# inferflow/inferflow

Measured on AMD Instinct MI355X. Metric: decode tokens/sec, Llama-2-7B Q4 batch=1 greedy (whole job), higher is better.
Workload: dtype i8 (Q8 activations x Q4_B32T1A weights, i32 dot, f32 scale, f16 I/O); 1 GPU; llama2_7b decode, Q4_B32T1A weights + F16 lm_head, F16 KV cache, batch 1 greedy, 16-token prompt, context 21..1851; parallelism=single, weights_bytes=4309647360

## Files before the change

inferflow_amd/csrc/ifa_decode_attn.h:

```cpp
#pragma once
#include "ifa_decode_kernels.h"

namespace ifa {

struct DecAttnParams {
    const half_t *q;
    const half_t *k_new;
    const half_t *v_new;
    uint8_t *kcache, *vcache;
    const int *state;
    const float *rope_tab;
    int heads, kv_heads, kv_q8;
    float kq_scale;
    int rope_order, rope_cols;
    int alibi, alibi_base, alibi_total;
    half_t *out;
    int max_ctx;
    int8_t *xq;
    long long *trace;
    const void *batch_rows;
    int q_stride;
};
struct DecAttnBatchRow { const uint8_t *kc, *vc; int n_ctx, pad; };

// ... 34 lines not shown
    float c[IFA_ATTN_NACC];
    __device__ __forceinline__ ScoreAcc() {
#pragma unroll
        for (int i = 0; i < IFA_ATTN_NACC; i++) c[i] = 0.0f;
    }
    __device__ __forceinline__ void add2(int p, half2_t q, half2_t k) {
        if constexpr (IFA_ATTN_NACC == 1) {
            c[0] = __builtin_fmaf((float)q[0], (float)k[0], c[0]);
            c[0] = __builtin_fmaf((float)q[1], (float)k[1], c[0]);
        } else {
            c[p % IFA_ATTN_NACC] = __builtin_amdgcn_fdot2(q, k, c[p % IFA_ATTN_NACC], false);
        }
    }
    __device__ __forceinline__ void add(int d, float q, float k) { c[d % IFA_ATTN_NACC] = __builtin_fmaf(q, k, c[d % IFA_ATTN_NACC]); }
    __device__ __forceinline__ float total() const {
        if constexpr (IFA_ATTN_NACC == 1) return c[0];
        else if constexpr (IFA_ATTN_NACC == 2) return c[0] + c[1];
        else if constexpr (IFA_ATTN_NACC == 4) return (c[0] + c[1]) + (c[2] + c[3]);
        else { float t = c[0]; for (int i = 1; i < IFA_ATTN_NACC; i++) t = t + c[i]; return t; }
    }
};

struct DecAttnFusedIn {
    const unsigned long long *gran;
    unsigned epoch;
    int pos;
    unsigned *err;
    long long timeout_ticks;
    unsigned long long *att_gran;
};

__host__ __device__ inline int att_gran_count(int heads, int hd) { return heads * hd / 4 + 2 * (heads * hd / 32) + heads; }

template <int HD, bool Q8, int PB, bool KT>
struct DecAttnRegs {
    static constexpr int DG = HD / 8, NSPLIT = 256 / DG, VPRE = PB / NSPLIT;
    static constexpr int KBYTES = (HD / 32) * 34;
    static constexpr int KALIGN = HD == 128 ? 8 : (HD == 64 ? 4 : 2);
    uint32_t kreg[Q8 ? 1 : HD / 2];
    uint32_t kq32[(Q8 && KALIGN >= 4) ? KBYTES / 4 : 1];
    uint16_t kq16[(Q8 && KALIGN < 4) ? KBYTES / 2 : 1];
    u32x4 kt[KT ? PB / NSPLIT : 1];
    u32x4 vreg[Q8 ? 1 : VPRE];
    uint32_t vqs[Q8 ? VPRE : 1], vqc[Q8 ? VPRE : 1][2];
    float rope_cs, rope_sn;
    half_t q_in, k_in, v_in;
};

template <int HD, bool Q8, bool BATCH, int PB, bool KT, bool FUSED, int PHASE = 0>
__device__ __forceinline__ void dec_attn_body(char *smem, const half_t *pq, const uint8_t *pkc, const uint8_t *pvc, int pheads, int pkvh,
                                              const DecAttnParams &P, const int h_in, const DecAttnFusedIn &F, DecAttnRegs<HD, Q8, PB, KT> &R)
{
    int pos_b = 0;
    if constexpr (FUSED) pos_b = F.pos;
    if constexpr (BATCH) {
        const DecAttnBatchRow br = reinterpret_cast<const DecAttnBatchRow *>(P.batch_rows)[blockIdx.y];
        pkc = br.kc; pvc = br.vc; pos_b = br.n_ctx - 1;
        pq += (size_t)blockIdx.y * P.q_stride;
    }
#define IFA_GP(T, p) ((const __attribute__((address_space(1))) T *)(p))
    uint8_t *const kcw = BATCH ? const_cast<uint8_t *>(pkc) : P.kcache;
    uint8_t *const vcw = BATCH ? const_cast<uint8_t *>(pvc) : P.vcache;
    const float *const rope_tab = BATCH ? P.rope_tab + (size_t)blockIdx.y * HD : P.rope_tab;
    half_t *const outp = BATCH ? P.out + (size_t)blockIdx.y * pheads * HD : P.out;
    static_assert(HD % 8 == 0 && HD <= 128 && (!Q8 || HD % 32 == 0), "head size: multiples of 8 up to 128 (Q8 rows: whole 32-blocks)");
    constexpr int DG = HD / 8;
    constexpr int NSPLIT = 256 / DG;
    half_t *qs = reinterpret_cast<half_t *>(smem);
    half_t *kn = qs + HD;
    half_t *vn = kn + HD;
    float *red = reinterpret_cast<float *>(vn + HD);
    float *opart = red + 16;
    static_assert(!KT || (!Q8 && !BATCH && (DG & (DG - 1)) == 0 && PB % NSPLIT == 0), "K tile through LDS: F16 rows, one query, power-of-two pieces per row");
    static_assert(!(FUSED && BATCH), "the fused tail is a single-query kernel");
    static_assert(PB >= NSPLIT && PB <= DEC_ATTN_MIN_ROWS, "prefetch bucket");
    uint8_t *ktile = reinterpret_cast<uint8_t *>(opart + NSPLIT * HD);
    half_t *S = reinterpret_cast<half_t *>(ktile + (KT ? (size_t)PB * HD * 2 : 0));
    const int h = h_in, tid = threadIdx.x, lane = tid & 63, wave = tid >> 6;
    const int group = pheads / pkvh;
    const int kvh = h / group;
    const bool writer = (h % group) == 0;
    const int kv_dim = pkvh * HD;
    const size_t row_bytes = Q8 ? (size_t)(kv_dim / 32) * 34 : (size_t)kv_dim * 2;
    const size_t head_off = Q8 ? (size_t)((kvh * HD) / 32) * 34 : (size_t)kvh * HD * 2;

    constexpr int KBYTES = (HD / 32) * 34;
    constexpr int KALIGN = HD == 128 ? 8 : (HD == 64 ? 4 : 2);
    auto &kreg = R.kreg; auto &kq32 = R.kq32; auto &kq16 = R.kq16; auto &kt = R.kt; auto &vreg = R.vreg; auto &vqs = R.vqs; auto &vqc = R.vqc;
    float &rope_cs = R.rope_cs, &rope_sn = R.rope_sn;
    half_t &q_in = R.q_in, &k_in = R.k_in, &v_in = R.v_in;
    auto load_k = [&](int j) {
        const uint8_t *rowp = pkc + (size_t)j * row_bytes + head_off;
        if constexpr (Q8) {
// ... 237 lines not shown
    if (n_ctx <= 64) {
        if (wave == 0) {
            if (tr) P.trace[h * 8 + 4] = wall_clock64();
            float e = 0.0f;
            if (tid < n_ctx) e = expf(P.kq_scale * h2f(S[tid]) - lmax);
            const float lsum0 = wave_sum(e);
            const float inv0 = 1.0f / (((lsum0 + 0.0f) + 0.0f) + 0.0f);
            if (tid < n_ctx) S[tid] = f2h(h2f(f2h(e)) * inv0);
        }
        __syncthreads();
    } else {
    if (lane == 0) red[wave] = lmax;
    __syncthreads();
    if (tr) P.trace[h * 8 + 4] = wall_clock64();
    const float mx = fmaxf(fmaxf(red[0], red[1]), fmaxf(red[2], red[3]));
    float lsum = 0.0f;
    for (int j = tid; j < n_ctx; j += 256) {
        const float e = expf(P.kq_scale * h2f(S[j]) - mx);
        lsum += e;
        S[j] = f2h(e);
    }
    lsum = wave_sum(lsum);
    if (lane == 0) red[4 + wave] = lsum;
    __syncthreads();
    const float inv = 1.0f / (((red[4] + red[5]) + red[6]) + red[7]);
    for (int j = tid; j < n_ctx; j += 256) S[j] = f2h(h2f(S[j]) * inv);
    __syncthreads();
    }
    if (tr) P.trace[h * 8 + 5] = wall_clock64();

    float o[8];
#pragma unroll
    for (int i = 0; i < 8; i++) o[i] = 0.0f;
    auto acc_v = [&](float pj, const u32x4 vv) {
        const half8_t v8 = __builtin_bit_cast(half8_t, vv);
#pragma unroll
        for (int e = 0; e < 8; e++) o[e] = __builtin_fmaf(pj, (float)v8[e], o[e]);
    };
    auto acc_new = [&](float pj) {
#pragma unroll
        for (int e = 0; e < 8; e++) o[e] = __builtin_fmaf(pj, h2f(vn[dg * 8 + e]), o[e]);
    };
    auto acc_q8w = [&](float pj, uint16_t scb, uint16_t c0, uint16_t c1, uint16_t c2, uint16_t c3) {
        const half_t sch = __builtin_bit_cast(half_t, scb);
        const half2_t sc2 = {sch, sch};
        half2_t v01, v23, v45, v67;
        q8x4_dequant_h((uint32_t)c0 | ((uint32_t)c1 << 16), sc2, v01, v23);
        q8x4_dequant_h((uint32_t)c2 | ((uint32_t)c3 << 16), sc2, v45, v67);
        o[0] = __builtin_fmaf(pj, (float)v01[0], o[0]); o[1] = __builtin_fmaf(pj, (float)v01[1], o[1]);
        o[2] = __builtin_fmaf(pj, (float)v23[0], o[2]); o[3] = __builtin_fmaf(pj, (float)v23[1], o[3]);
        o[4] = __builtin_fmaf(pj, (float)v45[0], o[4]); o[5] = __builtin_fmaf(pj, (float)v45[1], o[5]);
        o[6] = __builtin_fmaf(pj, (float)v67[0], o[6]); o[7] = __builtin_fmaf(pj, (float)v67[1], o[7]);
    };
    auto acc_q8 = [&](float pj, int j) {
        const auto *blk = IFA_GP(uint16_t, pvc + (size_t)j * row_bytes + head_off + (size_t)(dg / 4) * 34);
        typedef uint32_t u32x2_a2 __attribute__((ext_vector_type(2), aligned(2)));
        const u32x2_a2 cw = *IFA_GP(u32x2_a2, blk + 1 + (dg % 4) * 4);
        acc_q8w(pj, blk[0], (uint16_t)(cw[0] & 0xFFFFu), (uint16_t)(cw[0] >> 16), (uint16_t)(cw[1] & 0xFFFFu), (uint16_t)(cw[1] >> 16));
    };
#pragma unroll
    for (int i = 0; i < VPRE; i++) {
        const int j = sp + NSPLIT * i;
        if (j < n_ctx && vact) {
            const float pj = h2f(S[j]);
            if (j == pos) acc_new(pj);
            else if constexpr (Q8) acc_q8w(pj, (uint16_t)vqs[i], (uint16_t)(vqc[i][0] & 0xFFFFu), (uint16_t)(vqc[i][0] >> 16), (uint16_t)(vqc[i][1] & 0xFFFFu), (uint16_t)(vqc[i][1] >> 16));
            else acc_v(pj, vreg[i]);
        }
    }
    {
        constexpr int TB = 8;
        u32x4 tcur[Q8 ? 1 : TB], tnxt[Q8 ? 1 : TB];
        uint32_t ts_c[Q8 ? TB : 1], tc_c[Q8 ? TB : 1][2], ts_n[Q8 ? TB : 1], tc_n[Q8 ? TB : 1][2];
        const size_t tq_off = head_off + (size_t)(dg / 4) * 34;
        auto tload = [&](u32x4 (&dst)[Q8 ? 1 : TB], uint32_t (&ds)[Q8 ? TB : 1], uint32_t (&dc)[Q8 ? TB : 1][2], int j) {
#pragma unroll
            for (int u = 0; u < TB; u++) {
                const int jr = min(j + u * NSPLIT, n_ctx - 1);
                if constexpr (!Q8) dst[u] = IFA_GP(u32x4, pvc + (size_t)jr * row_bytes + head_off)[dg];
                else {
                    const auto *blk = IFA_GP(uint16_t, pvc + (size_t)jr * row_bytes + tq_off);
                    typedef uint32_t u32x2_a2 __attribute__((ext_vector_type(2), aligned(2)));
                    ds[u] = blk[0];
                    const u32x2_a2 cw = *IFA_GP(u32x2_a2, blk + 1 + (dg % 4) * 4);
                    dc[u][0] = cw[0]; dc[u][1] = cw[1];
                }
            }
        };
        int j = vact ? sp + NSPLIT * VPRE : n_ctx;
        if (j < n_ctx) tload(tcur, ts_c, tc_c, j);
        for (; j < n_ctx; j += TB * NSPLIT) {
            tload(tnxt, ts_n, tc_n, j + TB * NSPLIT);
#pragma unroll
            for (int u = 0; u < TB; u++) {
                const int jj = j + u * NSPLIT;
                if (jj >= n_ctx) break;
                const float pj = h2f(S[jj]);
                if (jj == pos) acc_new(pj);
                else if constexpr (Q8) acc_q8w(pj, (uint16_t)ts_c[u], (uint16_t)(tc_c[u][0] & 0xFFFFu), (uint16_t)(tc_c[u][0] >> 16), (uint16_t)(tc_c[u][1] & 0xFFFFu), (uint16_t)(tc_c[u][1] >> 16));
                else acc_v(pj, tcur[u]);
            }
#pragma unroll
            for (int u = 0; u < TB; u++) {
                if constexpr (Q8) { ts_c[u] = ts_n[u]; tc_c[u][0] = tc_n[u][0]; tc_c[u][1] = tc_n[u][1]; }
                else tcur[u] = tnxt[u];
            }
        }
    }
    if (vact) {
#pragma unroll
        for (int e = 0; e < 8; e++) opart[sp * HD + dg * 8 + e] = o[e];
    }
    if (tr) P.trace[h * 8 + 6] = wall_clock64();
    __syncthreads();
    if (tid < HD) {
        float acc = opart[tid];
        for (int s2 = 1; s2 < NSPLIT; s2++) acc = acc + opart[s2 * HD + tid];
        const half_t yh = f2h(acc);
        outp[(size_t)h * HD + tid] = yh;
        if constexpr (HD % 32 == 0 && !BATCH) { if (P.xq) dec_attn_emit_q8<HD>(P.xq, P.heads * HD, h, tid, yh); }
        if constexpr (FUSED && HD % 32 == 0) {
            if (F.att_gran) {
                const float val = h2f(yh);
                const float mxv = half_wave_max(fabsf(val));
                const float qsc = mxv / 127;
                const int qv = q8_round_div1(val, qsc);
                const int sum = half_wave_sum_i32(qv);
                const int q1 = dpp_xor1(qv), q2 = dpp_xor2(qv), q3 = dpp_xor1(q2);
                const unsigned long long tagw = (unsigned long long)F.epoch << 32;
                const int cols = pheads * HD, nc = cols / 4, nbk = cols / 32;
                if ((tid & 3) == 0) {
                    const uint32_t w4 = (uint32_t)(qv & 0xFF) | ((uint32_t)(q1 & 0xFF) << 8) | ((uint32_t)(q2 & 0xFF) << 16) | ((uint32_t)(q3 & 0xFF) << 24);
                    __hip_atomic_store(F.att_gran + (h * HD + tid) / 4, tagw | w4, __ATOMIC_RELAXED, __HIP_MEMORY_SCOPE_AGENT);
                }
                if ((tid & 31) == 0) {
                    const int blk = (h * HD + tid) >> 5;
                    __hip_atomic_store(F.att_gran + nc + blk, tagw | __builtin_bit_cast(uint32_t, h2f(f2h(qsc))), __ATOMIC_RELAXED, __HIP_MEMORY_SCOPE_AGENT);
                    __hip_atomic_store(F.att_gran + nc + nbk + blk, tagw | __builtin_bit_cast(uint32_t, (float)sum), __ATOMIC_RELAXED, __HIP_MEMORY_SCOPE_AGENT);
                }
                if (tid == 0) __hip_atomic_store(F.att_gran + nc + 2 * nbk + h, tagw | 1u, __ATOMIC_RELAXED, __HIP_MEMORY_SCOPE_AGENT);
            }
        }
    }
    if (tr) P.trace[h * 8 + 7] = wall_clock64();
}

template <int HD, bool Q8, bool BATCH = false, int PB = DEC_ATTN_MIN_ROWS, bool KT = false>
__global__ void __launch_bounds__(256) k_dec_attn(const half_t *pq, const uint8_t *pkc, const uint8_t *pvc, int pheads, int pkvh,
                                                  const DecAttnParams P)
{
    extern __shared__ __attribute__((aligned(16))) char smem[];
    DecAttnRegs<HD, Q8, PB, KT> R;
    dec_attn_body<HD, Q8, BATCH, PB, KT, false>(smem, pq, pkc, pvc, pheads, pkvh, P, (int)blockIdx.x, DecAttnFusedIn{}, R);
}

constexpr int DEC_ATTN_MAX_SPLITS = 32;

struct DecAttnSplitWs {
    half_t *S;
    float *lmax;
    float *opart;
    int nsplits;
};

__device__ __forceinline__ void dec_split_range(int n_ctx, int nsplits, int s, int &j0, int &j1)
{
    const int chunk = ((n_ctx + nsplits - 1) / nsplits + 63) / 64 * 64;
    j0 = min(s * chunk, n_ctx); j1 = min(j0 + chunk, n_ctx);
}

template <int HD, bool Q8>
__global__ void __launch_bounds__(256) k_dec_attn_scores(const DecAttnParams P, const DecAttnSplitWs ws)
{
    __shared__ __attribute__((aligned(16))) half_t qs[HD];
    __shared__ __attribute__((aligned(16))) half_t kn[HD];
// ... 316 lines not shown
```

inferflow_amd/csrc/ifa_decode_qkv_attn.h:

```cpp
#pragma once
#include "ifa_decode_kernels.h"
#include "ifa_decode_attn.h"

namespace ifa {

struct DecQkvAttnExtra {
    unsigned long long *gran;
    const unsigned *epoch;
    unsigned epoch_add;
    unsigned *err;
    int timeout_us;
    int gk;
    int unload;
};

#ifndef IFA_QA_EARLY_KV
#define IFA_QA_EARLY_KV 0
#endif
#ifndef IFA_QA_WARM_ROWS
#define IFA_QA_WARM_ROWS 1
#endif
constexpr int QA_THREADS = 512;

template <int DT, int NJ, int RW, int NORM, int HD, bool Q8, int PB, bool KT, int NP, bool UL = false>
// ... 109 lines not shown
    typename Fmt::X X;
    X.load(L.codes, L.scale, L.xsum, lane, g_nblk);
    {
        float a[RW];
#pragma unroll
        for (int i = 0; i < RW; i++) a[i] = w[i].dot(X);
#pragma unroll
        for (int i = 0; i < RW; i++) a[i] = wave_sum(a[i]);
        float a0 = 0.0f;
#pragma unroll
        for (int i = 0; i < RW; i++) { if (lane == i) a0 = a[i]; }
        const int lr = lane * WGV + lw;
        if (lane < RW && lr < RG) {
            const Row r = locate(lr);
            half_t y = dec_bias(a0, r.b, r.row);
            if (P.pre_scale != 0.0f) y = f2h(h2f(y) * P.pre_scale);
            r.y[r.row] = y;
            __hip_atomic_store(E.gran + r.vrow, ((unsigned long long)epoch << 32) | (unsigned long long)__builtin_bit_cast(uint16_t, y),
                               __ATOMIC_RELAXED, __HIP_MEMORY_SCOPE_AGENT);
        }
    }
    if (A.trace && threadIdx.x == 0) {
        A.trace[(size_t)(A.heads + (int)blockIdx.x) * 8 + 0] = t_kernel;
        A.trace[(size_t)(A.heads + (int)blockIdx.x) * 8 + 1] = wall_clock64();
    }
    if (attn_wg) {
        __syncthreads();
        if (wave >= 4) return;
        dec_attn_body<HD, Q8, false, PB, KT, true, IFA_QA_EARLY_KV ? 2 : 0>(smem, nullptr, A.kcache, A.vcache, A.heads, A.kv_heads, A, head, F, R);
        return;
    }
}

bool dec_qkv_attn_supported(int w_dtype, int cols, int heads, int kv_heads, int head_dim, int num_cus, int *gk_out, int *rw_out);
int dec_qkv_attn_launch(int w_dtype, int norm, bool kv_q8, int pb, bool kt, const DecGemvParams &P, const DecAttnParams &A, const DecQkvAttnExtra &E,
                        int max_ctx, hipStream_t s);
template <int DT>
int dec_qkv_attn_launch_dt(int norm, bool kv_q8, int pb, bool kt, int rw, const DecGemvParams &P, const DecAttnParams &A, const DecQkvAttnExtra &E,
                           int max_ctx, hipStream_t s);

}
```

inferflow_amd/csrc/ifa_dqkvattn_impl.h:

```cpp
#pragma once
#include "ifa_host.h"
#include "ifa_decode_qkv_attn.h"

namespace ifa {

template <int DT, int NJ, int RW, int NORM, bool Q8, int PB, bool KT, bool UL = false>
static int qa_go(const DecGemvParams &P, const DecAttnParams &A, const DecQkvAttnExtra &E, int max_ctx, hipStream_t s)
{
    constexpr int HD = 128;
    auto kern = k_dec_qkv_attn<DT, NJ, RW, NORM, HD, Q8, PB, KT, QA_THREADS / 128, UL>;
    const size_t smem = std::max(xlds_bytes(P.cols), dec_attn_smem(HD, max_ctx, KT ? PB : 0));
    if (smem > (size_t)160 * 1024) return ifa_fail(IFA_ERR_ARG, "fused QKV + attention: %zu bytes of LDS", smem);
    if (smem > 48 * 1024) IFA_HIP_CHECK(hipFuncSetAttribute((const void *)kern, hipFuncAttributeMaxDynamicSharedMemorySize, (int)smem));
    if (A.heads > 255 || A.kv_heads > 255 || E.gk > 0xFFFF) return ifa_fail(IFA_ERR_ARG, "fused QKV + attention: geometry exceeds the packed launch scalar");
    const int pgeo = A.heads | (A.kv_heads << 8) | (E.gk << 16);
    kern<<<dim3((unsigned)(A.kv_heads * E.gk)), dim3(QA_THREADS), smem, s>>>(P.x, P.norm_w, P.norm_b, P.cols, pgeo, P.W0[0], P.W0[1], P.W0[2], P, A, E);
    IFA_LAUNCH_CHECK();
    return IFA_OK;
}

template <int DT, int NJ, int RW, int NORM>
static int qa_pick(bool kv_q8, int pb, bool kt, const DecGemvParams &P, const DecAttnParams &A, const DecQkvAttnExtra &E, int max_ctx, hipStream_t s)
{
    if (kv_q8) {
        if (pb == 64) return qa_go<DT, NJ, RW, NORM, true, 64, false>(P, A, E, max_ctx, s);
        if (pb == 128) return qa_go<DT, NJ, RW, NORM, true, 128, false>(P, A, E, max_ctx, s);
        return qa_go<DT, NJ, RW, NORM, true, 256, false>(P, A, E, max_ctx, s);
    }
    if (kt) {
        if (pb == 64) return qa_go<DT, NJ, RW, NORM, false, 64, true>(P, A, E, max_ctx, s);
        if (pb == 128) return qa_go<DT, NJ, RW, NORM, false, 128, true>(P, A, E, max_ctx, s);
        return qa_go<DT, NJ, RW, NORM, false, 256, true>(P, A, E, max_ctx, s);
    }
    return qa_go<DT, NJ, RW, NORM, false, 256, false>(P, A, E, max_ctx, s);
}

template <int DT, int NJ, int RW, int NORM>
static int qa_pick_ul(bool kv_q8, int pb, bool kt, const DecGemvParams &P, const DecAttnParams &A, const DecQkvAttnExtra &E, int max_ctx, hipStream_t s)
{
    if (pb == 128) {
        if (kv_q8) return qa_go<DT, NJ, RW, NORM, true, 128, false, true>(P, A, E, max_ctx, s);
        if (kt) return qa_go<DT, NJ, RW, NORM, false, 128, true, true>(P, A, E, max_ctx, s);
    }
    if (kv_q8) return qa_go<DT, NJ, RW, NORM, true, 256, false, true>(P, A, E, max_ctx, s);
    if (kt) return qa_go<DT, NJ, RW, NORM, false, 256, true, true>(P, A, E, max_ctx, s);
    return qa_go<DT, NJ, RW, NORM, false, 256, false, true>(P, A, E, max_ctx, s);
}

template <int DT> constexpr int qa_nj(int cols) { return (cols / block_capacity(DT) + 63) / 64; }

template <int DT>
int dec_qkv_attn_launch_dt(int norm, bool kv_q8, int pb, bool kt, int rw, const DecGemvParams &P, const DecAttnParams &A, const DecQkvAttnExtra &E,
                           int max_ctx, hipStream_t s)
{
    constexpr int NJ4K = qa_nj<DT>(4096);
    const int nj = (P.nblk + 63) / 64;
    if (norm != 1) return ifa_fail(IFA_ERR_ARG, "fused QKV + attention: RMS-norm prologue only");
    if (E.unload && nj == NJ4K && rw == 6 && E.gk == 8) return qa_pick_ul<DT, NJ4K, 7, 1>(kv_q8, pb, kt, P, A, E, max_ctx, s);
    if (E.unload && nj == NJ4K && rw == 3 && E.gk == 32) return qa_pick_ul<DT, NJ4K, 4, 1>(kv_q8, pb, kt, P, A, E, max_ctx, s);
    if (nj == NJ4K && rw == 6) return qa_pick<DT, NJ4K, 6, 1>(kv_q8, pb, kt, P, A, E, max_ctx, s);
    if (nj == NJ4K && rw == 3) return qa_pick<DT, NJ4K, 3, 1>(kv_q8, pb, kt, P, A, E, max_ctx, s);
    return ifa_fail(IFA_ERR_ARG, "fused QKV + attention: no kernel for %d blocks per lane, %d rows per wave", nj, rw);
}

}
```

inferflow_amd/csrc/ifa_engine_decode.hip:

```cpp
#include "ifa_engine_state.h"

namespace ifae {

bool qkv_attn_layer_ok(const ifa_model *m, int l, int *gk_out);

static int attn_split_threshold(const ifa_model *m)
{
    if (m->opt_attn_split_ctx >= 0) return m->opt_attn_split_ctx;
    const ifa_model_config &c = m->cfg;
    bool tail = m->opt_attn_unload && m->opt_fuse_attn && waits_enabled() && dec_attn_smem(c.head_dim, c.max_ctx, 256) <= IFA_LDS_LIMIT;
    int gk = 0;
    for (int l = 0; tail && l < c.layers; l++) if (!qkv_attn_layer_ok(m, l, &gk)) tail = false;
    if (tail && (long long)c.kv_heads * gk > (long long)visible_cus()) tail = false;
    if (!tail) return 320;
    return c.heads > c.kv_heads ? 640 : 512;
}

void choose_attn_split(ifa_model *m, int reach)
{
    const int thr = attn_split_threshold(m);
    const int want = (thr > 0 && reach > thr) ? (reach > 8192 ? 16 : 8) : 0;
    if (want != m->attn_split) { m->attn_split = want; drop_graphs(m); }
    const int pb = reach <= 64 ? 64 : (reach <= 128 ? 128 : 256);
    if (pb != m->attn_pb) { m->attn_pb = pb; drop_graphs(m); }
}

__global__ void __launch_bounds__(256) k_touch(const uint8_t *__restrict__ p, size_t bytes, size_t stride, int *sink)
{
    size_t i = ((size_t)blockIdx.x * blockDim.x + threadIdx.x) * stride;
    int acc = 0;
    for (; i < bytes; i += (size_t)gridDim.x * blockDim.x * stride) acc += *reinterpret_cast<const int *>(p + i);
    if (acc == 0x7FFFFFFF) *sink = acc;
}

static long long *g_trace_ptr = nullptr;

bool fused_ok(const Tensor &t, bool long_rows)
{
    if (!t.present()) return false;
    if (fused_int8(t.dtype)) return t.tiled && (long_rows ? dec_gemv_supported_long(t.dtype, t.cols) : dec_gemv_supported(t.dtype, t.cols));
    return dec_gemv_h_supported(t.dtype, t.cols) && (long_rows || t.cols <= 8192);
}

template <int EPI, int NORM>
static int launch_dec_gemv(int w_dtype, const DecGemvParams &P, int wgs_per_cu_opt, hipStream_t s)
// ... 77 lines not shown
                }
        }
        const int ids_dense[] = {T_WQ, T_WK, T_WV, T_WO, T_W1, T_W2};
        const int ids_moe[] = {T_WQ, T_WK, T_WV, T_WO};
        const int *ids = moe ? ids_moe : ids_dense;
        const int n_ids = moe ? 4 : 6;
        for (int ii = 0; ii < n_ids; ii++) {
            const int id = ids[ii];
            const Tensor &t = L.t[id];
            if (!t.present()) return fail("fused path: a layer's weight matrix is missing");
            const bool plain_input = id == T_WO || id == T_W2;
            if (!fused_ok(t, plain_input)) return fail("fused GEMV: columns out of range for this weight format (or cols % 8 != 0 for fp16 activations)");
        }
        if (L.t[T_W3].present() && (!fused_ok(L.t[T_W3], false) || !same_fmt(L.t[T_W3].dtype, L.t[T_W1].dtype))) return fail("w1/w3 dtype mismatch");
        if (!L.t[T_ATTN_NORM].present()) return fail("pre-norm weights required");
        if (!L.t[T_FFN_NORM].present() && !c.parallel_attn) return fail("ffn pre-norm weights required");
    }
    const Tensor &lm = m->g[T_LM_HEAD];
    if (!lm.present()) {  }
    else if (lm.dtype == F16) {
        if (lm.cols > 8192 || lm.cols % 8 != 0) return fail("fused F16 lm_head needs cols <= 8192");
    } else if (!fused_ok(lm, false) || !m->g[T_OUT_NORM].present()) {
        return fail("fused lm_head: columns out of range for its weight format (or no output norm)");
    }
    if (m->g[T_EMBD].present() && m->g[T_EMBD].dtype != F16) return fail("F16 embeddings required");
    return true;
}

int sep_norm(ifa_model *m, const half_t *x, const Tensor &w, const Tensor &b, half_t *dst)
{
    return ifa_layernorm(m->cfg.norm_kind, x, 1, (size_t)m->cfg.dim, w.data, b.data, 0.0f, m->cfg.eps, dst, (ifa_stream)m->stream);
}

bool qkv_attn_layer_ok(const ifa_model *m, int l, int *gk_out)
{
    const ifa_model_config &c = m->cfg;
    const Layer &L = m->layers[(size_t)l];
    if (c.norm_kind != 0 || c.tp_size > 1) return false;
    const Tensor &wq = L.t[T_WQ], &wk = L.t[T_WK], &wv = L.t[T_WV];
    if (!wq.present() || !wk.present() || !wv.present() || !wq.tiled || !wk.tiled || !wv.tiled) return false;
    if (!fused_int8(wq.dtype) || !same_fmt(wq.dtype, wk.dtype) || !same_fmt(wq.dtype, wv.dtype)) return false;
    if ((int)wq.rows != c.heads * c.head_dim || (int)wk.rows != c.kv_heads * c.head_dim || (int)wv.rows != c.kv_heads * c.head_dim) return false;
    int rw = 0;
    return dec_qkv_attn_supported(wq.dtype, (int)wq.cols, c.heads, c.kv_heads, c.head_dim, num_cus(), gk_out, &rw);
}

int qkv_attn_ready(ifa_model *m)
{
    const ifa_model_config &c = m->cfg;
    int want = m->opt_fuse_attn && waits_enabled() && !m->attn_split && dec_attn_smem(c.head_dim, c.max_ctx, 256) <= IFA_LDS_LIMIT;
    int gk = 0;
    for (int l = 0; want && l < c.layers; l++) if (!qkv_attn_layer_ok(m, l, &gk)) want = 0;
    if (want && (long long)c.kv_heads * gk > (long long)visible_cus()) want = 0;
    if (want && !m->qa_gran) {
        const size_t n = (size_t)c.layers * (size_t)(c.heads + 2 * c.kv_heads) * c.head_dim;
        IFA_HIP_CHECK(hipMalloc((void **)&m->qa_gran, n * 8));
        IFA_HIP_CHECK(hipMemsetAsync(m->qa_gran, 0, n * 8, m->stream));
        if (m->qa_call) { (void)hipFree(m->qa_call); m->qa_call = nullptr; }
        if (m->qa_err) { (void)hipFree(m->qa_err); m->qa_err = nullptr; }
        IFA_HIP_CHECK(hipMalloc((void **)&m->qa_call, 16));
        IFA_HIP_CHECK(hipMemsetAsync(m->qa_call, 0, 16, m->stream));
        IFA_HIP_CHECK(hipMalloc((void **)&m->qa_err, 16));
        IFA_HIP_CHECK(hipMemsetAsync(m->qa_err, 0, 16, m->stream));
        IFA_HIP_CHECK(hipStreamSynchronize(m->stream));
    }
    int want_ch = (m->opt_fuse_ffn && waits_enabled() && c.norm_kind == 0 && c.tp_size <= 1 && c.experts == 0
                   && !c.parallel_attn && !c.share_input && num_cus() <= visible_cus()) ? std::min(m->opt_fuse_ffn, 2) : 0;
    if (want_ch == 2 && (!m->attq || !m->opt_attn_q8 || c.head_dim % 32 != 0)) want_ch = 1;
    for (int l = 0; want_ch && l < c.layers; l++) {
        const Layer &L = m->layers[(size_t)l];
        const Tensor &wo = L.t[T_WO], &w1 = L.t[T_W1], &w3 = L.t[T_W3], &w2 = L.t[T_W2];
        if (!w1.present() || !w1.tiled || !w3.present() || !w3.tiled || !w2.present() || !w2.tiled || !L.t[T_FFN_NORM].present()
            || (int)w1.cols != c.dim || (int)w2.rows != c.dim || w2.cols != w1.rows || w3.rows != w1.rows || !same_fmt(w1.dtype, w3.dtype)
            || !dec_chain_supported(w1.dtype, w2.dtype, w1.dtype, c.dim, (int)w1.rows, false, c.dim, num_cus()))
            want_ch = 0;
        else if (want_ch == 2 && (!wo.present() || !wo.tiled || (int)wo.rows != c.dim
                                  || !dec_chain_supported(w1.dtype, w2.dtype, wo.dtype, c.dim, (int)w1.rows, true, (int)wo.cols, num_cus())))
// ... 667 lines not shown
```

inferflow_amd/csrc/ifa_engine_state.h:

```cpp
#pragma once
#include <chrono>
#include <cstdlib>
#include <cstring>
#include <map>
#include <string>
#include <vector>
#include "ifa_host.h"
#include "ifa_decode_kernels.h"
#include "ifa_decode_attn.h"
#include "ifa_decode_gemv.h"
#include "ifa_moe.h"
#include "ifa_gemm_rows_mfma.h"
#include "ifa_gemm_big.h"
#include "ifa_decode_lmhead_tail.h"
#include "ifa_decode_singles.h"
#include "ifa_decode_qkv_attn.h"
#include "ifa_decode_chain.h"

using namespace ifa;

namespace ifae {


enum { T_EMBD = 0, T_OUT_NORM = 1, T_OUT_NORM_B = 2, T_LM_HEAD = 3,
// ... 190 lines not shown
                             float partial_rotary_factor, ifa_stream stream);

static inline const uint8_t *rows_w(const ifa_model *m, const Tensor &t) { return (const uint8_t *)(m->opt_rows_mo && t.mo ? t.mo : t.tiled); }

static inline int rows_mo(const ifa_model *m, const Tensor &t) { return m->opt_rows_mo && t.mo ? 1 : 0; }

namespace ifae {

void drop_graphs(ifa_model *m);
int perf_begin(ifa_model *m, int key);
void perf_end(ifa_model *m, int idx);
int perf_collect(ifa_model *m);
struct PerfSpan {
    ifa_model *m; int idx;
    PerfSpan(ifa_model *mm, int key, bool on = true) : m(mm), idx(on ? perf_begin(mm, key) : -1) {}
    ~PerfSpan() { done(); }
    void done() { if (idx >= 0) { perf_end(m, idx); idx = -1; } }
};
void free_tensor(Tensor &t);
void *kv_ptr(ifa_model *m, size_t layer, int slot, bool is_v);
int ensure_mo(ifa_model *m);
int ensure_mo_build(ifa_model *m);
int ensure_x32(ifa_model *m);
int ensure_q3hn(ifa_model *m);
int ensure_scratch(ifa_model *m, int T);
void choose_attn_split(ifa_model *m, int reach);
bool fused_ok(const Tensor &t, bool long_rows);
int lmhead_grid(const DecLmHeadParams &P, int wgs_per_cu_opt);
int launch_lmhead(const DecLmHeadParams &P, int norm, int wgs_per_cu_opt, hipStream_t s, const DecStepTail *Z = nullptr);
bool has_post_norms(const ifa_model *m);
bool fused_supported(const ifa_model *m, std::string *why);
int sep_norm(ifa_model *m, const half_t *x, const Tensor &w, const Tensor &b, half_t *dst);
void attn_params(ifa_model *m, int l, DecAttnParams &A);
bool qkv_attn_layer_ok(const ifa_model *m, int l, int *gk_out);
int qkv_attn_ready(ifa_model *m);
void qkv_params(ifa_model *m, int l, const half_t *x, DecGemvParams &P);
int launch_qkv_attn(ifa_model *m, int l, const half_t *x, unsigned tag_add = 0);
int launch_qkv(ifa_model *m, int l, const half_t *x);
int launch_attn(ifa_model *m, int l);
int launch_wo(ifa_model *m, int l, const half_t *x, half_t *partial = nullptr);
void moe_params(ifa_model *m, Layer &L, DecGemvParams &P, int slot, int tab_off);
int launch_ffn13(ifa_model *m, int l, int moe_slot = -1, const half_t *x_layer = nullptr, int moe_nslots = 1);
int launch_w2(ifa_model *m, int l, half_t *xnext, half_t *partial = nullptr, int moe_slot = -1, bool moe_last = false,
                     const half_t *residual2 = nullptr, int moe_t1_slot = 0);
int launch_chain(ifa_model *m, int l, const half_t *x, half_t *xnext, unsigned tag_add = 0);
bool step_tail_ok(const ifa_model *m);
DecLmHeadParams lm_params(ifa_model *m, const half_t *x, half_t *logits_out);
int step_tail_ready(ifa_model *m);
int launch_lm_tail(ifa_model *m, const half_t *x);
int launch_gather(ifa_model *m);
int launch_lm(ifa_model *m, const half_t *x, half_t *logits_out = nullptr);
int enqueue_fused_step(ifa_model *m);
int decode_impl(ifa_model *m, int first_token, int start_pos, int n_steps, int *out_tokens_host, float *elapsed_ms, bool prepare_only);
int gather_rows(ifa_model *m, const half_t *src, const int *idx_dev, int T, int dim, int n_src, half_t *dst, float scale);
int matmul(ifa_model *m, const half_t *A, int T, const Tensor &W, const Tensor &bias, half_t *C);
int norm_rows(ifa_model *m, const half_t *x, int T, const Tensor &w, const Tensor &b, half_t *y, float base = 0.0f);
int ffn_dense(ifa_model *m, const half_t *x, int T, const Tensor &w1, const Tensor &b1, const Tensor &w3, const Tensor &b3,
                     const Tensor &w2, const Tensor &b2, half_t *out, int perf_base = 0);
int layer_tail_ops(ifa_model *m, int l, int T, half_t *&x, const half_t *attn_in, bool &xn_ready);
int forward_ops(ifa_model *m, const int *tokens_host, int T, int prefix_len, void *logits_out, int *next_token, bool no_head = false);
bool batch_fused_ok(const ifa_model *m, int n);
bool prefill_big_ok(const ifa_model *m);
bool prefill_mid_ok(ifa_model *m, int T, bool any_length);
int batch_fused_layer(ifa_model *m, int l, int n, const half_t *x, half_t *xnext, const void *rows_l);
int forward_batch(ifa_model *m, int n, const int *tokens_host, const int *pos_host, const int *slot_host, int *next_tokens,
                         void *logits_out);
int pool_enqueue(ifa_model *m, const half_t *logits, int n_rows);
// ... 23 lines not shown
```

Measured before the change: 621.8 tokens/s.

## Add single-wave short-context attention path for fused tail when position under 64

Adds a specialized attention body for the fused QKV+attention kernel used when the context is shorter than 64 rows. Scores and softmax are done in one wave with shuffles instead of LDS reductions, and K/V are prefetched in a fixed small count. This is meant to cut sync and reduction overhead on early decode steps. It also restricts the attention-split threshold to configurations the unload kernels actually support, and factors the output store into a shared helper. Only steps with position under 64 take the new path, which is a small share of a run reaching context 1851, so any effect is limited to those steps.

Result: no change. 619.8 tokens/s (-0.3%).

```diff
diff --git a/inferflow_amd/csrc/ifa_decode_attn.h b/inferflow_amd/csrc/ifa_decode_attn.h
--- a/inferflow_amd/csrc/ifa_decode_attn.h
+++ b/inferflow_amd/csrc/ifa_decode_attn.h
@@ -90,6 +90,36 @@
 
 __host__ __device__ inline int att_gran_count(int heads, int hd) { return heads * hd / 4 + 2 * (heads * hd / 32) + heads; }
 
+template <int HD, bool BATCH, bool FUSED>
+__device__ __forceinline__ void dec_attn_store_out(float acc, half_t *outp, int h, int tid, int pheads, const DecAttnParams &P, const DecAttnFusedIn &F)
+{
+    const half_t yh = f2h(acc);
+    outp[(size_t)h * HD + tid] = yh;
+    if constexpr (HD % 32 == 0 && !BATCH) { if (P.xq) dec_attn_emit_q8<HD>(P.xq, P.heads * HD, h, tid, yh); }
+    if constexpr (FUSED && HD % 32 == 0) {
+        if (F.att_gran) {
+            const float val = h2f(yh);
+            const float mxv = half_wave_max(fabsf(val));
+            const float qsc = mxv / 127;
+            const int qv = q8_round_div1(val, qsc);
+            const int sum = half_wave_sum_i32(qv);
+            const int q1 = dpp_xor1(qv), q2 = dpp_xor2(qv), q3 = dpp_xor1(q2);
+            const unsigned long long tagw = (unsigned long long)F.epoch << 32;
+            const int cols = pheads * HD, nc = cols / 4, nbk = cols / 32;
+            if ((tid & 3) == 0) {
+                const uint32_t w4 = (uint32_t)(qv & 0xFF) | ((uint32_t)(q1 & 0xFF) << 8) | ((uint32_t)(q2 & 0xFF) << 16) | ((uint32_t)(q3 & 0xFF) << 24);
+                __hip_atomic_store(F.att_gran + (h * HD + tid) / 4, tagw | w4, __ATOMIC_RELAXED, __HIP_MEMORY_SCOPE_AGENT);
+            }
+            if ((tid & 31) == 0) {
+                const int blk = (h * HD + tid) >> 5;
+                __hip_atomic_store(F.att_gran + nc + blk, tagw | __builtin_bit_cast(uint32_t, h2f(f2h(qsc))), __ATOMIC_RELAXED, __HIP_MEMORY_SCOPE_AGENT);
+                __hip_atomic_store(F.att_gran + nc + nbk + blk, tagw | __builtin_bit_cast(uint32_t, (float)sum), __ATOMIC_RELAXED, __HIP_MEMORY_SCOPE_AGENT);
+            }
+            if (tid == 0) __hip_atomic_store(F.att_gran + nc + 2 * nbk + h, tagw | 1u, __ATOMIC_RELAXED, __HIP_MEMORY_SCOPE_AGENT);
+        }
+    }
+}
+
 template <int HD, bool Q8, int PB, bool KT>
 struct DecAttnRegs {
     static constexpr int DG = HD / 8, NSPLIT = 256 / DG, VPRE = PB / NSPLIT;
@@ -105,10 +135,282 @@
     half_t q_in, k_in, v_in;
 };
 
+#define IFA_GP(T, p) ((const __attribute__((address_space(1))) T *)(p))
+
+__device__ __forceinline__ void pv_acc_f16(float (&o)[8], float pj, const u32x4 vv)
+{
+    const half8_t v8 = __builtin_bit_cast(half8_t, vv);
+#pragma unroll
+    for (int e = 0; e < 8; e++) o[e] = __builtin_fmaf(pj, (float)v8[e], o[e]);
+}
+__device__ __forceinline__ void pv_acc_q8(float (&o)[8], float pj, uint16_t scb, uint16_t c0, uint16_t c1, uint16_t c2, uint16_t c3)
+{
+    const half_t sch = __builtin_bit_cast(half_t, scb);
+    const half2_t sc2 = {sch, sch};
+    half2_t v01, v23, v45, v67;
+    q8x4_dequant_h((uint32_t)c0 | ((uint32_t)c1 << 16), sc2, v01, v23);
+    q8x4_dequant_h((uint32_t)c2 | ((uint32_t)c3 << 16), sc2, v45, v67);
+    o[0] = __builtin_fmaf(pj, (float)v01[0], o[0]); o[1] = __builtin_fmaf(pj, (float)v01[1], o[1]);
+    o[2] = __builtin_fmaf(pj, (float)v23[0], o[2]); o[3] = __builtin_fmaf(pj, (float)v23[1], o[3]);
+    o[4] = __builtin_fmaf(pj, (float)v45[0], o[4]); o[5] = __builtin_fmaf(pj, (float)v45[1], o[5]);
+    o[6] = __builtin_fmaf(pj, (float)v67[0], o[6]); o[7] = __builtin_fmaf(pj, (float)v67[1], o[7]);
+}
+
+template <int HD, bool Q8, int PB, bool KT>
+__device__ __forceinline__ void dec_attn_short_body(char *smem, const uint8_t *pkc, const uint8_t *pvc, int pheads, int pkvh,
+                                                    const DecAttnParams &P, const int h, const DecAttnFusedIn &F)
+{
+    static_assert(HD == 128, "short tail: the fused launch's head size");
+    constexpr int DG = HD / 8, NSPLIT = 256 / DG, NK = 64 / NSPLIT;
+    constexpr int KBYTES = (HD / 32) * 34;
+    static_assert(PB >= 64, "the K tile holds at least 64 rows");
+    half_t *qs = reinterpret_cast<half_t *>(smem);
+    half_t *kn = qs + HD;
+    half_t *vn = kn + HD;
+    float *red = reinterpret_cast<float *>(vn + HD);
+    float *opart = red + 16;
+    uint8_t *ktile = reinterpret_cast<uint8_t *>(opart + NSPLIT * HD);
+    half_t *S = reinterpret_cast<half_t *>(ktile + (KT ? (size_t)PB * HD * 2 : 0));
+    const int tid = threadIdx.x, lane = tid & 63, wave = __builtin_amdgcn_readfirstlane(tid >> 6);
+    const int pos = F.pos, n_ctx = pos + 1;
+    const int group = pheads / pkvh, kvh = h / group;
+    const bool writer = (h % group) == 0;
+    const int kv_dim = pkvh * HD;
+    const size_t row_bytes = Q8 ? (size_t)(kv_dim / 32) * 34 : (size_t)kv_dim * 2;
+    const size_t head_off = Q8 ? (size_t)((kvh * HD) / 32) * 34 : (size_t)kvh * HD * 2;
+    const int dg = tid % DG, sp = tid / DG;
+    const bool tr = P.trace != nullptr && tid == 0;
+
+    uint32_t kreg[Q8 ? 1 : HD / 2];
+    uint32_t kq32[Q8 ? KBYTES / 4 : 1];
+    u32x4 kt[KT ? NK : 1];
+    u32x4 vreg[Q8 ? 1 : NK];
+    uint32_t vqs[Q8 ? NK : 1], vqc[Q8 ? NK : 1][2];
+    if constexpr (KT) {
+#pragma unroll
+        for (int i = 0; i < NK; i++) kt[i] = IFA_GP(u32x4, pkc + (size_t)min(sp + NSPLIT * i, pos) * row_bytes + head_off)[dg];
+    } else if (wave == 0) {
+        const uint8_t *rowp = pkc + (size_t)min(lane, pos) * row_bytes + head_off;
+        if constexpr (Q8) {
+#pragma unroll
+            for (int i = 0; i < KBYTES / 8; i++) { const u32x2 t = IFA_GP(u32x2, rowp)[i]; kq32[2 * i] = t[0]; kq32[2 * i + 1] = t[1]; }
+        } else {
+#pragma unroll
+            for (int i = 0; i < HD / 8; i++) {
+                const u32x4 t = IFA_GP(u32x4, rowp)[i];
+                kreg[4 * i] = t[0]; kreg[4 * i + 1] = t[1]; kreg[4 * i + 2] = t[2]; kreg[4 * i + 3] = t[3];
+            }
+        }
+    }
+    const int d = min(tid, HD - 1);
+    const bool o2 = P.rope_order == 2;
+    const int hc = P.rope_cols / 2;
+    const bool rot = P.rope_order != 0 && (!o2 || d < 2 * hc);
+    const bool first = o2 ? d < hc : (d & 1) == 0;
+    const int pair = o2 ? (d < hc ? d : d - hc) : d >> 1;
+    const int dp = !rot ? d : (o2 ? (first ? d + hc : d - hc) : (d ^ 1));
+    float rope_cs = 1.0f, rope_sn = 0.0f;
+    {
+        const float *rt = P.rope_tab ? P.rope_tab : reinterpret_cast<const float *>(F.gran);
+        typedef float f32x2 __attribute__((ext_vector_type(2)));
+        const f32x2 cs = *IFA_GP(f32x2, rt + 2 * (rot ? pair : 0));
+        if (rot) { rope_cs = cs[0]; rope_sn = cs[1]; }
+    }
+#pragma unroll
+    for (int i = 0; i < NK; i++) {
+        const int j = min(sp + NSPLIT * i, pos);
+        if constexpr (!Q8) {
+            vreg[i] = IFA_GP(u32x4, pvc + (size_t)j * row_bytes + head_off)[dg];
+        } else {
+            const auto *blk = IFA_GP(uint16_t, pvc + (size_t)j * row_bytes + head_off + (size_t)(dg / 4) * 34);
+            typedef uint32_t u32x2_a2 __attribute__((ext_vector_type(2), aligned(2)));
+            vqs[i] = blk[0];
+            const u32x2_a2 cw = *IFA_GP(u32x2_a2, blk + 1 + (dg % 4) * 4);
+            vqc[i][0] = cw[0]; vqc[i][1] = cw[1];
+        }
+    }
+    if (tr) P.trace[h * 8 + 0] = wall_clock64();
+
+    if (tid < HD) {
+        const unsigned long long *gq = F.gran + (size_t)h * HD, *gk = F.gran + (size_t)(pheads + kvh) * HD,
+                                 *gv = F.gran + (size_t)(pheads + pkvh + kvh) * HD;
+        half_t q_in = (half_t)0, k_in = (half_t)0, v_in = (half_t)0, qp_in = (half_t)0, kp_in = (half_t)0;
+        const long long t_give_up = wall_clock64() + F.timeout_ticks;
+        for (;;) {
+            const unsigned long long a = __hip_atomic_load(gq + d, __ATOMIC_RELAXED, __HIP_MEMORY_SCOPE_AGENT);
+            const unsigned long long b = __hip_atomic_load(gk + d, __ATOMIC_RELAXED, __HIP_MEMORY_SCOPE_AGENT);
+            const unsigned long long c = __hip_atomic_load(gv + d, __ATOMIC_RELAXED, __HIP_MEMORY_SCOPE_AGENT);
+            const unsigned long long ap = __hip_atomic_load(gq + dp, __ATOMIC_RELAXED, __HIP_MEMORY_SCOPE_AGENT);
+            const unsigned long long bp = __hip_atomic_load(gk + dp, __ATOMIC_RELAXED, __HIP_MEMORY_SCOPE_AGENT);
+            const bool ok = (unsigned)(a >> 32) == F.epoch && (unsigned)(b >> 32) == F.epoch && (unsigned)(c >> 32) == F.epoch
+                         && (unsigned)(ap >> 32) == F.epoch && (unsigned)(bp >> 32) == F.epoch;
+            q_in = __builtin_bit_cast(half_t, (uint16_t)a); k_in = __builtin_bit_cast(half_t, (uint16_t)b); v_in = __builtin_bit_cast(half_t, (uint16_t)c);
+            qp_in = __builtin_bit_cast(half_t, (uint16_t)ap); kp_in = __builtin_bit_cast(half_t, (uint16_t)bp);
+            if (__all(ok)) break;
+            if (wall_clock64() > t_give_up) { if (lane == 0) atomicExch(F.err, 0x51u); break; }
+            __builtin_amdgcn_s_sleep(2);
+        }
+        if (tr) P.trace[h * 8 + 1] = wall_clock64();
+        auto rotate = [&](half_t own, half_t partner) -> half_t {
+            const float x0 = h2f(first ? own : partner), x1 = h2f(first ? partner : own);
+            const float a = x0 * rope_cs, bq = x1 * rope_sn, dd = x0 * rope_sn, e = x1 * rope_cs;
+            const half_t r0 = f2h(a - bq), r1 = f2h(dd + e);
+            return rot ? (first ? r0 : r1) : own;
+        };
+        half_t q_r = rotate(q_in, qp_in), k_r = rotate(k_in, kp_in), v_r = v_in;
+        if constexpr (Q8) {
+            auto round_trip = [&](half_t x, uint8_t *cache) -> half_t {
+                const float val = h2f(x);
+                const float mx = half_wave_max(fabsf(val));
+                const float sc = mx / 127;
+                int qv = sc <= 0.000001f ? 0 : (int)roundf(val / sc);
+                qv = min(max(qv, -128), 127);
+                const half_t sch = f2h(sc);
+                if (writer) {
+                    uint8_t *blk = cache + (size_t)pos * row_bytes + head_off + (size_t)(tid >> 5) * 34;
+                    blk[2 + (tid & 31)] = (uint8_t)(int8_t)qv;
+                    if ((tid & 31) == 0) *reinterpret_cast<uint16_t *>(blk) = __builtin_bit_cast(uint16_t, sch);
+                }
+                return f2h((float)qv * h2f(sch));
+            };
+            k_r = round_trip(k_r, P.kcache);
+            v_r = round_trip(v_r, P.vcache);
+        } else if (writer) {
+            reinterpret_cast<half_t *>(P.kcache + (size_t)pos * row_bytes + head_off)[tid] = k_r;
+            reinterpret_cast<half_t *>(P.vcache + (size_t)pos * row_bytes + head_off)[tid] = v_r;
+        }
+        qs[tid] = q_r; kn[tid] = k_r; vn[tid] = v_r;
+    }
+    if constexpr (KT) {
+#pragma unroll
+        for (int i = 0; i < NK; i++) {
+            const int j = sp + NSPLIT * i;
+            *reinterpret_cast<u32x4 *>(ktile + ((size_t)j * DG + (size_t)(dg ^ (j & (DG - 1)))) * 16) = kt[i];
+        }
+    }
+    __syncthreads();
+    if (tr) P.trace[h * 8 + 2] = wall_clock64();
+
+    const u32x4 vnew = reinterpret_cast<const u32x4 *>(vn)[dg];
+    uint32_t pbits = 0;
+    if (KT || wave == 0) {
+        uint32_t qr[HD / 2];
+#pragma unroll
+        for (int i = 0; i < HD / 8; i++) {
+            const u32x4 t = reinterpret_cast<const u32x4 *>(qs)[i];
+            qr[4 * i] = t[0]; qr[4 * i + 1] = t[1]; qr[4 * i + 2] = t[2]; qr[4 * i + 3] = t[3];
+        }
+        const bool is_new = lane == pos;
+        ScoreAcc acc;
+        if constexpr (!Q8) {
+            if constexpr (KT) {
+#pragma unroll
+                for (int i = 0; i < DG; i++) {
+                    const uint8_t *src = is_new ? reinterpret_cast<const uint8_t *>(kn) + i * 16
+                                                : ktile + ((size_t)lane * DG + (size_t)(i ^ (lane & (DG - 1)))) * 16;
+                    const u32x4 t = *reinterpret_cast<const u32x4 *>(src);
+                    kreg[4 * i] = t[0]; kreg[4 * i + 1] = t[1]; kreg[4 * i + 2] = t[2]; kreg[4 * i + 3] = t[3];
+                }
+            } else if (is_new) {
+#pragma unroll
+                for (int i = 0; i < HD / 8; i++) {
+                    const u32x4 t = reinterpret_cast<const u32x4 *>(kn)[i];
+                    kreg[4 * i] = t[0]; kreg[4 * i + 1] = t[1]; kreg[4 * i + 2] = t[2]; kreg[4 * i + 3] = t[3];
+                }
+            }
+            if (tr) P.trace[h * 8 + 3] = wall_clock64();
+#pragma unroll
+            for (int i = 0; i < HD / 2; i++) acc.add2(i, __builtin_bit_cast(half2_t, qr[i]), __builtin_bit_cast(half2_t, kreg[i]));
+        } else {
+            if (tr) P.trace[h * 8 + 3] = wall_clock64();
+            if (is_new) {
+                uint32_t knr[HD / 2];
+#pragma unroll
+                for (int i = 0; i < HD / 8; i++) {
+                    const u32x4 t = reinterpret_cast<const u32x4 *>(kn)[i];
+                    knr[4 * i] = t[0]; knr[4 * i + 1] = t[1]; knr[4 * i + 2] = t[2]; knr[4 * i + 3] = t[3];
+                }
+#pragma unroll
+                for (int i = 0; i < HD / 2; i++) acc.add2(i, __builtin_bit_cast(half2_t, qr[i]), __builtin_bit_cast(half2_t, knr[i]));
+            } else {
+#pragma unroll
+                for (int b = 0; b < HD / 32; b++) {
+                    const uint32_t sw = kq32[(b * 34) >> 2] >> (8 * ((b * 34) & 3));
+                    const half_t sch = __builtin_bit_cast(half_t, (uint16_t)(sw & 0xFFFFu));
+                    const half2_t sc2 = {sch, sch};
+#pragma unroll
+                    for (int w4 = 0; w4 < 8; w4++) {
+                        const int B0 = b * 34 + 2 + 4 * w4;
+                        const uint32_t cw = (B0 & 3) == 0 ? kq32[B0 >> 2]
+                            : __builtin_amdgcn_alignbyte(kq32[(B0 >> 2) + 1 < KBYTES / 4 ? (B0 >> 2) + 1 : (B0 >> 2)], kq32[B0 >> 2], (B0 & 3));
+                        half2_t lo, hi;
+                        q8x4_dequant_h(cw, sc2, lo, hi);
+                        acc.add2(2 * w4, __builtin_bit_cast(half2_t, qr[b * 16 + 2 * w4]), lo);
+                        acc.add2(2 * w4 + 1, __builtin_bit_cast(half2_t, qr[b * 16 + 2 * w4 + 1]), hi);
+                    }
+                }
+            }
+        }
+        const float alpha = 1.0f / sqrtf((float)HD) / P.kq_scale;
+        half_t s = f2h(alpha * acc.total());
+        if (P.alibi) { const float a = (float)lane * alibi_slope(h + P.alibi_base, P.alibi_total); s = f2h(a + h2f(s)); }
+        if (tr) P.trace[h * 8 + 4] = wall_clock64();
+        const bool live = lane < n_ctx;
+        const float lmax = wave_max(live ? P.kq_scale * h2f(s) : -INFINITY);
+        float e = 0.0f;
+        if (live) e = expf(P.kq_scale * h2f(s) - lmax);
+        const float lsum0 = wave_sum(e);
+        const float inv0 = 1.0f / (((lsum0 + 0.0f) + 0.0f) + 0.0f);
+        const half_t p = f2h(h2f(f2h(e)) * inv0);
+        pbits = __builtin_bit_cast(uint16_t, p);
+        if constexpr (!KT) { if (live) S[lane] = p; }
+    }
+    if constexpr (!KT) __syncthreads();
+    if (tr) P.trace[h * 8 + 5] = wall_clock64();
+
+    float o[8];
+#pragma unroll
+    for (int i = 0; i < 8; i++) o[i] = 0.0f;
+#pragma unroll
+    for (int i = 0; i < NK; i++) {
+        const int j = sp + NSPLIT * i;
+        half_t pj_h;
+        if constexpr (KT) pj_h = __builtin_bit_cast(half_t, (uint16_t)__shfl((int)pbits, j));
+        else pj_h = S[min(j, pos)];
+        if (j < n_ctx) {
+            const float pj = h2f(pj_h);
+            if constexpr (!Q8) {
+                pv_acc_f16(o, pj, j == pos ? vnew : vreg[i]);
+            } else {
+                if (j == pos) pv_acc_f16(o, pj, vnew);
+                else pv_acc_q8(o, pj, (uint16_t)vqs[i], (uint16_t)(vqc[i][0] & 0xFFFFu), (uint16_t)(vqc[i][0] >> 16), (uint16_t)(vqc[i][1] & 0xFFFFu), (uint16_t)(vqc[i][1] >> 16));
+            }
+        }
+    }
+    typedef float f32x4 __attribute__((ext_vector_type(4)));
+    *reinterpret_cast<f32x4 *>(opart + sp * HD + dg * 8) = f32x4{o[0], o[1], o[2], o[3]};
+    *reinterpret_cast<f32x4 *>(opart + sp * HD + dg * 8 + 4) = f32x4{o[4], o[5], o[6], o[7]};
+    if (tr) P.trace[h * 8 + 6] = wall_clock64();
+    __syncthreads();
+    if (tid < HD) {
+        float part[NSPLIT];
+#pragma unroll
+        for (int s2 = 0; s2 < NSPLIT; s2++) part[s2] = opart[s2 * HD + tid];
+        float acc = part[0];
+#pragma unroll
+        for (int s2 = 1; s2 < NSPLIT; s2++) acc = acc + part[s2];
+        dec_attn_store_out<HD, false, true>(acc, P.out, h, tid, pheads, P, F);
+    }
+    if (tr) P.trace[h * 8 + 7] = wall_clock64();
+}
+
 template <int HD, bool Q8, bool BATCH, int PB, bool KT, bool FUSED, int PHASE = 0>
 __device__ __forceinline__ void dec_attn_body(char *smem, const half_t *pq, const uint8_t *pkc, const uint8_t *pvc, int pheads, int pkvh,
                                               const DecAttnParams &P, const int h_in, const DecAttnFusedIn &F, DecAttnRegs<HD, Q8, PB, KT> &R)
 {
+    if constexpr (FUSED && PHASE == 0 && HD == 128) {
+        if (F.pos < 64) { dec_attn_short_body<HD, Q8, PB, KT>(smem, pkc, pvc, pheads, pkvh, P, h_in, F); return; }
+    }
     int pos_b = 0;
     if constexpr (FUSED) pos_b = F.pos;
     if constexpr (BATCH) {
@@ -116,7 +418,6 @@
         pkc = br.kc; pvc = br.vc; pos_b = br.n_ctx - 1;
         pq += (size_t)blockIdx.y * P.q_stride;
     }
-#define IFA_GP(T, p) ((const __attribute__((address_space(1))) T *)(p))
     uint8_t *const kcw = BATCH ? const_cast<uint8_t *>(pkc) : P.kcache;
     uint8_t *const vcw = BATCH ? const_cast<uint8_t *>(pvc) : P.vcache;
     const float *const rope_tab = BATCH ? P.rope_tab + (size_t)blockIdx.y * HD : P.rope_tab;
@@ -420,26 +721,12 @@
     float o[8];
 #pragma unroll
     for (int i = 0; i < 8; i++) o[i] = 0.0f;
-    auto acc_v = [&](float pj, const u32x4 vv) {
-        const half8_t v8 = __builtin_bit_cast(half8_t, vv);
-#pragma unroll
-        for (int e = 0; e < 8; e++) o[e] = __builtin_fmaf(pj, (float)v8[e], o[e]);
-    };
+    auto acc_v = [&](float pj, const u32x4 vv) { pv_acc_f16(o, pj, vv); };
     auto acc_new = [&](float pj) {
 #pragma unroll
         for (int e = 0; e < 8; e++) o[e] = __builtin_fmaf(pj, h2f(vn[dg * 8 + e]), o[e]);
     };
-    auto acc_q8w = [&](float pj, uint16_t scb, uint16_t c0, uint16_t c1, uint16_t c2, uint16_t c3) {
-        const half_t sch = __builtin_bit_cast(half_t, scb);
-        const half2_t sc2 = {sch, sch};
-        half2_t v01, v23, v45, v67;
-        q8x4_dequant_h((uint32_t)c0 | ((uint32_t)c1 << 16), sc2, v01, v23);
-        q8x4_dequant_h((uint32_t)c2 | ((uint32_t)c3 << 16), sc2, v45, v67);
-        o[0] = __builtin_fmaf(pj, (float)v01[0], o[0]); o[1] = __builtin_fmaf(pj, (float)v01[1], o[1]);
-        o[2] = __builtin_fmaf(pj, (float)v23[0], o[2]); o[3] = __builtin_fmaf(pj, (float)v23[1], o[3]);
-        o[4] = __builtin_fmaf(pj, (float)v45[0], o[4]); o[5] = __builtin_fmaf(pj, (float)v45[1], o[5]);
-        o[6] = __builtin_fmaf(pj, (float)v67[0], o[6]); o[7] = __builtin_fmaf(pj, (float)v67[1], o[7]);
-    };
+    auto acc_q8w = [&](float pj, uint16_t scb, uint16_t c0, uint16_t c1, uint16_t c2, uint16_t c3) { pv_acc_q8(o, pj, scb, c0, c1, c2, c3); };
     auto acc_q8 = [&](float pj, int j) {
         const auto *blk = IFA_GP(uint16_t, pvc + (size_t)j * row_bytes + head_off + (size_t)(dg / 4) * 34);
         typedef uint32_t u32x2_a2 __attribute__((ext_vector_type(2), aligned(2)));
@@ -504,31 +791,7 @@
     if (tid < HD) {
         float acc = opart[tid];
         for (int s2 = 1; s2 < NSPLIT; s2++) acc = acc + opart[s2 * HD + tid];
-        const half_t yh = f2h(acc);
-        outp[(size_t)h * HD + tid] = yh;
-        if constexpr (HD % 32 == 0 && !BATCH) { if (P.xq) dec_attn_emit_q8<HD>(P.xq, P.heads * HD, h, tid, yh); }
-        if constexpr (FUSED && HD % 32 == 0) {
-            if (F.att_gran) {
-                const float val = h2f(yh);
-                const float mxv = half_wave_max(fabsf(val));
-                const float qsc = mxv / 127;
-                const int qv = q8_round_div1(val, qsc);
-                const int sum = half_wave_sum_i32(qv);
-                const int q1 = dpp_xor1(qv), q2 = dpp_xor2(qv), q3 = dpp_xor1(q2);
-                const unsigned long long tagw = (unsigned long long)F.epoch << 32;
-                const int cols = pheads * HD, nc = cols / 4, nbk = cols / 32;
-                if ((tid & 3) == 0) {
-                    const uint32_t w4 = (uint32_t)(qv & 0xFF) | ((uint32_t)(q1 & 0xFF) << 8) | ((uint32_t)(q2 & 0xFF) << 16) | ((uint32_t)(q3 & 0xFF) << 24);
-                    __hip_atomic_store(F.att_gran + (h * HD + tid) / 4, tagw | w4, __ATOMIC_RELAXED, __HIP_MEMORY_SCOPE_AGENT);
-                }
-                if ((tid & 31) == 0) {
-                    const int blk = (h * HD + tid) >> 5;
-                    __hip_atomic_store(F.att_gran + nc + blk, tagw | __builtin_bit_cast(uint32_t, h2f(f2h(qsc))), __ATOMIC_RELAXED, __HIP_MEMORY_SCOPE_AGENT);
-                    __hip_atomic_store(F.att_gran + nc + nbk + blk, tagw | __builtin_bit_cast(uint32_t, (float)sum), __ATOMIC_RELAXED, __HIP_MEMORY_SCOPE_AGENT);
-                }
-                if (tid == 0) __hip_atomic_store(F.att_gran + nc + 2 * nbk + h, tagw | 1u, __ATOMIC_RELAXED, __HIP_MEMORY_SCOPE_AGENT);
-            }
-        }
+        dec_attn_store_out<HD, BATCH, FUSED>(acc, outp, h, tid, pheads, P, F);
     }
     if (tr) P.trace[h * 8 + 7] = wall_clock64();
 }
diff --git a/inferflow_amd/csrc/ifa_decode_qkv_attn.h b/inferflow_amd/csrc/ifa_decode_qkv_attn.h
--- a/inferflow_amd/csrc/ifa_decode_qkv_attn.h
+++ b/inferflow_amd/csrc/ifa_decode_qkv_attn.h
@@ -165,6 +165,7 @@
     }
 }
 
+inline bool dec_qkv_attn_unloads(int gk, int rw) { return (rw == 6 && gk == 8) || (rw == 3 && gk == 32); }
 bool dec_qkv_attn_supported(int w_dtype, int cols, int heads, int kv_heads, int head_dim, int num_cus, int *gk_out, int *rw_out);
 int dec_qkv_attn_launch(int w_dtype, int norm, bool kv_q8, int pb, bool kt, const DecGemvParams &P, const DecAttnParams &A, const DecQkvAttnExtra &E,
                         int max_ctx, hipStream_t s);
diff --git a/inferflow_amd/csrc/ifa_dqkvattn_impl.h b/inferflow_amd/csrc/ifa_dqkvattn_impl.h
--- a/inferflow_amd/csrc/ifa_dqkvattn_impl.h
+++ b/inferflow_amd/csrc/ifa_dqkvattn_impl.h
@@ -56,8 +56,8 @@
     constexpr int NJ4K = qa_nj<DT>(4096);
     const int nj = (P.nblk + 63) / 64;
     if (norm != 1) return ifa_fail(IFA_ERR_ARG, "fused QKV + attention: RMS-norm prologue only");
-    if (E.unload && nj == NJ4K && rw == 6 && E.gk == 8) return qa_pick_ul<DT, NJ4K, 7, 1>(kv_q8, pb, kt, P, A, E, max_ctx, s);
-    if (E.unload && nj == NJ4K && rw == 3 && E.gk == 32) return qa_pick_ul<DT, NJ4K, 4, 1>(kv_q8, pb, kt, P, A, E, max_ctx, s);
+    if (E.unload && nj == NJ4K && dec_qkv_attn_unloads(E.gk, rw) && rw == 6) return qa_pick_ul<DT, NJ4K, 7, 1>(kv_q8, pb, kt, P, A, E, max_ctx, s);
+    if (E.unload && nj == NJ4K && dec_qkv_attn_unloads(E.gk, rw) && rw == 3) return qa_pick_ul<DT, NJ4K, 4, 1>(kv_q8, pb, kt, P, A, E, max_ctx, s);
     if (nj == NJ4K && rw == 6) return qa_pick<DT, NJ4K, 6, 1>(kv_q8, pb, kt, P, A, E, max_ctx, s);
     if (nj == NJ4K && rw == 3) return qa_pick<DT, NJ4K, 3, 1>(kv_q8, pb, kt, P, A, E, max_ctx, s);
     return ifa_fail(IFA_ERR_ARG, "fused QKV + attention: no kernel for %d blocks per lane, %d rows per wave", nj, rw);
diff --git a/inferflow_amd/csrc/ifa_engine_decode.hip b/inferflow_amd/csrc/ifa_engine_decode.hip
--- a/inferflow_amd/csrc/ifa_engine_decode.hip
+++ b/inferflow_amd/csrc/ifa_engine_decode.hip
@@ -2,15 +2,13 @@
 
 namespace ifae {
 
-bool qkv_attn_layer_ok(const ifa_model *m, int l, int *gk_out);
-
 static int attn_split_threshold(const ifa_model *m)
 {
     if (m->opt_attn_split_ctx >= 0) return m->opt_attn_split_ctx;
     const ifa_model_config &c = m->cfg;
     bool tail = m->opt_attn_unload && m->opt_fuse_attn && waits_enabled() && dec_attn_smem(c.head_dim, c.max_ctx, 256) <= IFA_LDS_LIMIT;
-    int gk = 0;
-    for (int l = 0; tail && l < c.layers; l++) if (!qkv_attn_layer_ok(m, l, &gk)) tail = false;
+    int gk = 0, rw = 0;
+    for (int l = 0; tail && l < c.layers; l++) if (!qkv_attn_layer_ok(m, l, &gk, &rw) || !dec_qkv_attn_unloads(gk, rw)) tail = false;
     if (tail && (long long)c.kv_heads * gk > (long long)visible_cus()) tail = false;
     if (!tail) return 320;
     return c.heads > c.kv_heads ? 640 : 512;
@@ -154,7 +152,7 @@
     return ifa_layernorm(m->cfg.norm_kind, x, 1, (size_t)m->cfg.dim, w.data, b.data, 0.0f, m->cfg.eps, dst, (ifa_stream)m->stream);
 }
 
-bool qkv_attn_layer_ok(const ifa_model *m, int l, int *gk_out)
+bool qkv_attn_layer_ok(const ifa_model *m, int l, int *gk_out, int *rw_out)
 {
     const ifa_model_config &c = m->cfg;
     const Layer &L = m->layers[(size_t)l];
@@ -164,7 +162,7 @@
     if (!fused_int8(wq.dtype) || !same_fmt(wq.dtype, wk.dtype) || !same_fmt(wq.dtype, wv.dtype)) return false;
     if ((int)wq.rows != c.heads * c.head_dim || (int)wk.rows != c.kv_heads * c.head_dim || (int)wv.rows != c.kv_heads * c.head_dim) return false;
     int rw = 0;
-    return dec_qkv_attn_supported(wq.dtype, (int)wq.cols, c.heads, c.kv_heads, c.head_dim, num_cus(), gk_out, &rw);
+    return dec_qkv_attn_supported(wq.dtype, (int)wq.cols, c.heads, c.kv_heads, c.head_dim, num_cus(), gk_out, rw_out ? rw_out : &rw);
 }
 
 int qkv_attn_ready(ifa_model *m)
diff --git a/inferflow_amd/csrc/ifa_engine_state.h b/inferflow_amd/csrc/ifa_engine_state.h
--- a/inferflow_amd/csrc/ifa_engine_state.h
+++ b/inferflow_amd/csrc/ifa_engine_state.h
@@ -246,7 +246,7 @@
 bool fused_supported(const ifa_model *m, std::string *why);
 int sep_norm(ifa_model *m, const half_t *x, const Tensor &w, const Tensor &b, half_t *dst);
 void attn_params(ifa_model *m, int l, DecAttnParams &A);
-bool qkv_attn_layer_ok(const ifa_model *m, int l, int *gk_out);
+bool qkv_attn_layer_ok(const ifa_model *m, int l, int *gk_out, int *rw_out = nullptr);
 int qkv_attn_ready(ifa_model *m);
 void qkv_params(ifa_model *m, int l, const half_t *x, DecGemvParams &P);
 int launch_qkv_attn(ifa_model *m, int l, const half_t *x, unsigned tag_add = 0);
```
